# Xneonz0/JPEG-DSP-Studio

Measured on AMD Instinct MI355X. Metric: Mpixels/s forward+inverse pipeline @ Q=50 4:2:0; PSNR vs ref, higher is better.
Workload: dtype f32+f64; 1 GPU; 1920x1080 RGB, Q=50, 4:2:0, prefilter=on, 8x8 blocks (BASELINE configs[1]); global_batch_frames=64, pipeline=serial forward then inverse per step, parallelism=frame-shard x1, world_size=1, quant_table=local (one rank)

## Files before the change

include/jds.h:

```cpp
#ifndef JDS_H
#define JDS_H

#include <stdint.h>

#ifdef __cplusplus
extern "C" {
#endif

#define JDS_ABI_VERSION 3

#define JDS_OK       0
#define JDS_EINVAL  (-1)
#define JDS_ENOTSUP (-2)
#define JDS_EHIP    (-3)
#define JDS_ENOMEM  (-4)

#define JDS_SS_444 0
#define JDS_SS_422 1
#define JDS_SS_420 2
#define JDS_SS_GRAY 3

#define JDS_RUN_SSE 1u
#define JDS_RUN_FWD 2u
#define JDS_RUN_INV 4u
// ... 327 lines not shown
  int64_t rgb_off;
  int64_t H, W;
  int32_t quality;
  int32_t subsampling;
} jds_rgb_item;
int jds_jpeg_quality_info(int32_t quality, int32_t subsampling, int64_t H, int64_t W, jds_jpeg_info* out);
int jds_jpeg_forward_dev(jds_ctx* ctx, const jds_jpeg_info* info, const uint8_t* rgb_dev, int16_t* coeffs_dev,
                         void* stream);
int jds_rgb_to_jpeg(jds_ctx* ctx, const uint8_t* rgb, int32_t rgb_on_device, int64_t H, int64_t W, int32_t quality,
                    int32_t subsampling, int32_t optimize, uint8_t* out, int64_t out_cap, int64_t* out_len);
int jds_rgb_batch_to_jpeg(jds_ctx* ctx, const uint8_t* rgb_base, int32_t rgb_on_device, const jds_rgb_item* items_in,
                          int32_t n, int32_t optimize, uint8_t* out, int64_t out_cap, int32_t out_on_device,
                          jds_jpeg_transcode_item* items_out, int64_t* out_bytes);
int jds_selftest_jpeg_forward(const jds_jpeg_info* info, const uint8_t* rgb, int16_t* coeffs_out);
int jds_selftest_jpeg_fwd_quant(int32_t q, int32_t n, int32_t* out, int32_t* bound);

int jds_selftest_huffdec(const uint8_t* data, int64_t len, int32_t subseq_bits, int16_t* coeffs, int64_t coeffs_cap,
                         int32_t* rounds_out);

int jds_selftest_dct8x8(const double* in, double* out, int64_t n, int32_t inverse);
int jds_selftest_dct16x16(const double* in, double* out, int64_t n, int32_t inverse);

int jds_selftest_fwd32(int32_t subsampling, int32_t prefilter, const double* gauss, const uint8_t* rgb, int64_t H,
                       int64_t W, int32_t plane, int32_t rows_first, float* coeffs, double* bound);
int jds_selftest_fwd16(int32_t subsampling, int32_t prefilter, const double* gauss, const uint8_t* rgb, int64_t H,
                       int64_t W, int32_t plane, int32_t rows_first, float* coeffs, double* bound);

int jds_selftest_inv_fast(int32_t subsampling, const int16_t* coeffs, const double* qtable, int64_t H, int64_t W,
                          int32_t fuse, double* values, uint8_t* bytes);

int jds_selftest_inv_fast16(int32_t subsampling, const int16_t* coeffs, const double* qtable, int64_t H, int64_t W,
                            int32_t fuse, double* values, uint8_t* bytes);

int jds_selftest_inv_rows(int32_t subsampling, int64_t H, int32_t ty, int32_t* out, uint8_t* need);

int jds_selftest_area_tab(int32_t src, int32_t dst, int32_t* n, int32_t* si, double* a);

#ifdef __cplusplus
}
#endif

#endif
```

jpeg-dsp-studio_amd/csrc/jds_abi.hip:

```cpp
#include <algorithm>
#include <mutex>
#include <new>
#include <string>

#include "jds_abi.hpp"
#include "jds_dct16.hpp"
#include "jds_dct8.hpp"

#ifdef JDS_INV6
#define JDS_INV6_LIST 1
#else
#define JDS_INV6_LIST 0
#endif

static const double SSIM_C1 = (0.01 * 255) * (0.01 * 255);
static const double SSIM_C2 = (0.03 * 255) * (0.03 * 255);

thread_local char g_err[512] = "";

constexpr int SSIM_ROWS_MIN = 32;
constexpr size_t SSIM_SCRATCH = (size_t)16 << 30;

static int run_ssim_batch(jds_ctx* c, int items, const uint8_t* const* a, const uint8_t* const* b, int H, int W,
                          double* out, int out_stride, unsigned long long* sse) {
// ... 204 lines not shown

static void fill_geometry(const Geo& G, int mode, jds_geometry* o) {
  o->H = G.H;
  o->W = G.W;
  o->chroma_h = G.hc;
  o->chroma_w = G.wc;
  o->y_blocks_y = G.nby;
  o->y_blocks_x = G.nbx;
  o->c_blocks_y = G.ncy;
  o->c_blocks_x = G.ncx;
  o->coeffs_per_frame = G.cpf;
  o->cb_offset = G.off_cb;
  o->cr_offset = G.off_cr;
  o->tiles = G.tiles_y * G.tiles_x;
  if (G.bs == 16) {
    int my, mx;
    o->threads_fwd = tile_dims16(mode, &my, &mx);
    o->threads_inv = 256;
  } else {
    o->threads_fwd = mode == JDS_SS_420 ? Cfg<M420>::TF : mode == JDS_SS_422 ? Cfg<M422>::TF : Cfg<M444>::TF;
    o->threads_inv = Cfg<M420>::TI;
  }
  o->reserved = 0;
}

static void make_fq(const jds_params* p, FrameQ* q) {
  q->qmax = 0.0;
  q->pad_ = 0.0;
  for (int i = 0; i < 64; ++i) {
    q->q[i] = p->qtable[i];
    q->q16[i] = 16.0 * p->qtable[i];
    q->qmax = q->qmax > p->qtable[i] ? q->qmax : p->qtable[i];
  }
}

static int gen_prepare(const Geo& g, int n_frames, int n, DevBuf& tab, DevBuf& sub, DevBuf& rec, hipStream_t s) {
  const size_t nt = (size_t)g.hc + g.wc;
  AreaTap* h = (AreaTap*)malloc(sizeof(AreaTap) * nt);
  if (!h) return fail(JDS_ENOMEM, "host allocation failed");
  if (area_tab_build(g.H, g.hc, h) < 0 || area_tab_build(g.W, g.wc, h + g.hc) < 0) {
    free(h);
    return fail(JDS_EINVAL, "INTER_AREA table with more than 4 taps per sample (%dx%d)", g.H, g.W);
  }
  hipError_t e = tab.ensure(sizeof(AreaTap) * nt);
  if (e == hipSuccess) e = hipMemcpyAsync(tab.p, h, sizeof(AreaTap) * nt, hipMemcpyHostToDevice, s);
  if (e == hipSuccess) e = hipStreamSynchronize(s);
  free(h);
  HIP_TRY(e);
  HIP_TRY(sub.ensure(sizeof(double) * gen_sub_doubles(g) * (size_t)n_frames));
  HIP_TRY(rec.ensure(sizeof(double) * gen_rec_doubles(g) * (size_t)n));
  return JDS_OK;
}


extern "C" {

int jds_abi_version(void) { return JDS_ABI_VERSION; }

const char* jds_last_error(void) { return g_err; }

int jds_device_count(int* n) {
  if (!n) return fail(JDS_EINVAL, "null argument");
  int c = 0;
  hipError_t e = hipGetDeviceCount(&c);
  if (e != hipSuccess) {
    *n = 0;
// ... 1290 lines not shown
                       int64_t W, int32_t plane, int32_t rows_first, float* coeffs, double* bound) {
  if (!gauss || !rgb || !coeffs || !bound || H < 1 || W < 1 || H > 4096 || W > 4096 || plane < 0 || plane > 2 ||
      subsampling < JDS_SS_444 || subsampling > JDS_SS_420)
    return fail(JDS_EINVAL, "bad argument");
  const bool pf = prefilter != 0 && subsampling != JDS_SS_444;
  double E[512];
  fast_fwd16_bounds(subsampling, pf, gauss, E);
  memcpy(bound, E + (plane ? 256 : 0), 256 * sizeof(double));
  if (fwd16_host_plane(subsampling, pf, gauss, rgb, (int)H, (int)W, plane, rows_first, coeffs))
    return fail(JDS_EINVAL, "plane size must be a multiple of 16");
  return JDS_OK;
}

int jds_selftest_inv_fast(int32_t subsampling, const int16_t* coeffs, const double* qtable, int64_t H, int64_t W,
                          int32_t fuse, double* values, uint8_t* bytes) {
  if (!coeffs || !qtable || !values || !bytes || H < 1 || W < 1 || H > 4096 || W > 4096 ||
      subsampling < JDS_SS_444 || subsampling > JDS_SS_420)
    return fail(JDS_EINVAL, "bad argument");
  if (inv_fast_host(subsampling, coeffs, qtable, (int)H, (int)W, fuse, 8, values, bytes))
    return fail(JDS_EINVAL, "odd chroma geometry: the certified inverse runs even sizes only");
  return JDS_OK;
}

int jds_selftest_inv_fast16(int32_t subsampling, const int16_t* coeffs, const double* qtable, int64_t H, int64_t W,
                            int32_t fuse, double* values, uint8_t* bytes) {
  if (!coeffs || !qtable || !values || !bytes || H < 1 || W < 1 || H > 4096 || W > 4096 ||
      subsampling < JDS_SS_444 || subsampling > JDS_SS_420)
    return fail(JDS_EINVAL, "bad argument");
  if (inv_fast_host(subsampling, coeffs, qtable, (int)H, (int)W, fuse, 16, values, bytes))
    return fail(JDS_EINVAL, "odd chroma geometry: the certified inverse runs even sizes only");
  return JDS_OK;
}

int jds_selftest_area_tab(int32_t src, int32_t dst, int32_t* n, int32_t* si, double* a) {
  if (src < 1 || dst < 1 || dst > src || !n || !si || !a) return fail(JDS_EINVAL, "bad argument");
  AreaTap* t = (AreaTap*)malloc(sizeof(AreaTap) * (size_t)dst);
  if (!t) return fail(JDS_ENOMEM, "host allocation failed");
  if (area_tab_build(src, dst, t) < 0) {
    free(t);
    return fail(JDS_EINVAL, "more than 4 taps per sample");
  }
  for (int d = 0; d < dst; ++d) {
    n[d] = t[d].n;
    for (int k = 0; k < 4; ++k) {
      si[4 * d + k] = k < t[d].n ? t[d].si[k] : -1;
      a[4 * d + k] = k < t[d].n ? t[d].a[k] : 0.0;
    }
  }
  free(t);
  return JDS_OK;
}

int jds_selftest_inv_rows(int32_t subsampling, int64_t H, int32_t ty, int32_t* out, uint8_t* need) {
  if (!out || H < 1 || H > 65536 || ty < 0 || subsampling < JDS_SS_444 || subsampling > JDS_SS_420)
    return fail(JDS_EINVAL, "bad argument");
  int o[8];
  inv_rows(subsampling, (int)H, ty, o);
  for (int i = 0; i < 8; ++i) out[i] = o[i];
  if (need)
    for (int i = 0; i < o[5]; ++i)
      for (int r = 0; r < 8; ++r) need[8 * i + r] = (uint8_t)inv_rows_need(subsampling, (int)H, ty, o[4] + i, r);
  return JDS_OK;
}

int jds_selftest_dct16x16(const double* in, double* out, int64_t n, int32_t inverse) {
  if (!in || !out || n < 0) return fail(JDS_EINVAL, "bad argument");
// ... 18 lines not shown
```

jpeg-dsp-studio_amd/csrc/jds_internal.hpp:

```cpp
#pragma once
#include <hip/hip_runtime.h>
#include <stdint.h>

#include "jds.h"

namespace jds {

enum Mode : int { M444 = JDS_SS_444, M422 = JDS_SS_422, M420 = JDS_SS_420 };

struct Geo {
  int H, W;
  int hc, wc;
  int nby, nbx;
  int ncy, ncx;
  int nmy, nmx;
  int tiles_y, tiles_x, ty_off, tx_off;
  long long cpf;
  long long off_cb, off_cr;
  double up_sy, up_sx;
  int bs;
  int gen;
  int afx, afy;
  int inv_yoff;
};
// ... 16 lines not shown
  int si[4];
  int pad;
  double a[4];
};

struct GenBufs {
  const AreaTap* tabs;
  double* sub;
  double* rec;
};

__host__ __device__ inline int fix_wpi(const Geo& g) { return (int)((g.cpf / 64 + 31) / 32); }

struct Fwd16Fast {
  const void* fq16;
  const float* gk32;
  uint32_t* part;
  uint2* fixlist;
  unsigned* counters;
  int fix_all;
  int parity;
};

struct InvFix {
  unsigned* count;
  unsigned* item;
  int fix_all;
  int parity;
  int rot;
  int probe;
  uint2* list;
};

struct FrameQ {
  double q16[64];
  double q[64];
  double qmax;
  double pad_;
};

template <int MODE>
struct Cfg {
  static constexpr int SY = (MODE == M420) ? 2 : 1;
  static constexpr int SX = (MODE == M444) ? 1 : 2;
  static constexpr int MH = 8 * SY, MW = 8 * SX;
  static constexpr int TH = (MODE == M444) ? 16 : 32;
  static constexpr int TW = 64;
  static constexpr int MY = TH / MH, MX = TW / MW;
  static constexpr int YBR = TH / 8, YBC = TW / 8;
  static constexpr int CBR = TH / MH, CBC = TW / MW;
  static constexpr int NYB = YBR * YBC, NCB = CBR * CBC;
  static constexpr int NB = NYB + 2 * NCB;
  static constexpr int TF = NB * 8;
  static constexpr int RY = (SY == 2) ? 1 : 0, RX = (SX == 2) ? 1 : 0;
  static constexpr int RBR = CBR + 2 * RY, RBC = CBC + 2 * RX;
  static constexpr int NRB = RBR * RBC;
  static constexpr int CWR = 8 * CBR + 2 * RY;
  static constexpr int CWC = 8 * CBC + 2 * RX;
  static constexpr int TI = 384;
};

struct KMarks {
  hipEvent_t* ev = nullptr;
  char (*name)[64] = nullptr;
  int n = 0, cap = 0;
  long long dropped = 0;
};
extern thread_local KMarks* t_kmarks;
void kmark(hipStream_t s, const char* fmt, ...) __attribute__((format(printf, 2, 3)));

__device__ inline void finalize_frame(const Geo& g, jds_frame_stats* s, int zero_bin) {
// ... 34 lines not shown
```

jpeg-dsp-studio_amd/csrc/jds_inv_common.hpp:

```cpp
#pragma once
#include <hip/hip_runtime.h>
#include <stdint.h>

#include "jds_internal.hpp"


namespace jds {

template <int MODE>
struct Inv {
  static constexpr int SY = Cfg<MODE>::SY, SX = Cfg<MODE>::SX;
  static constexpr int TH = (MODE == M420) ? 64 : 32;
  static constexpr int TW = (MODE == M444) ? 64 : 128;
  static constexpr int NT = (MODE == M444) ? 256 : 512;
  static constexpr int RY = (SY == 2) ? 1 : 0, RX = (SX == 2) ? 1 : 0;
  static constexpr int YBC = TW / 8, NYB = (TH / 8) * YBC;
  static constexpr int RB = NT / 8;
  static constexpr int CBR = TH / (8 * SY) + 2 * RY, CBC = TW / (8 * SX) + 2 * RX;
  static constexpr int NCB = CBR * CBC;
  static constexpr int CWR = TH / SY + 2 * RY, CWC = TW / SX + 2 * RX;
  static constexpr int CWS = SX == 2 ? CWC + 4 : CWC;
  static constexpr int NROW = (CBR - 2 * RY) * CBC * 8 + 2 * RY * CBC;
  static constexpr int MB = NCB > RB ? NCB : RB;
  static constexpr int WPE = (MODE == M444) ? 3 : 4;
  static_assert(NCB * 8 <= NT && NROW <= NT && NYB % RB == 0, "one round per chroma plane");
};

template <int MODE>
struct InvRows {
  int y0, cby0, ncbr, cwy0;
  __host__ __device__ __forceinline__ InvRows(int ty, int yoff) {
    using I = Inv<MODE>;
    y0 = ty * I::TH - yoff;
    cby0 = ty * (I::TH / (8 * I::SY)) - I::RY;
    ncbr = I::CBR - (yoff ? 1 : 0);
    cwy0 = y0 / I::SY - I::RY;
  }
  __host__ __device__ __forceinline__ bool need(int by, int r) const {
    return !Inv<MODE>::RY || (unsigned)(by * 8 + r - cwy0) < (unsigned)Inv<MODE>::CWR;
  }
};

constexpr int MS = 72;

__device__ __forceinline__ int tslot(int r, int c) { return r * 8 + ((((c >> 1) ^ (r & 3)) << 1) | (c & 1)); }

struct Col16 {
  int16_t q[8];
};
__device__ __forceinline__ Col16 load_col(const int16_t* __restrict__ plane, long long boff, int v, bool ok) {
  const int16_t* blk = plane + (ok ? boff : 0ll);
  Col16 c;
#pragma unroll
  for (int r = 0; r < 8; ++r) c.q[r] = blk[r * 8 + v];
  return c;
}

#ifdef JDS_INV6
typedef short jds_short2 __attribute__((ext_vector_type(2)));
struct Col16p {
  jds_short2 w[4];
  __device__ __forceinline__ int q(int r) const { return (int)((r & 1) ? w[r >> 1].y : w[r >> 1].x); }
};
__device__ __forceinline__ Col16p load_colp(const int16_t* __restrict__ plane, long long boff, int v, bool ok) {
  const int16_t* blk = plane + (ok ? boff : 0ll);
  Col16p c;
#pragma unroll
  for (int i = 0; i < 4; ++i) {
    c.w[i].x = blk[(2 * i) * 8 + v];
    c.w[i].y = blk[(2 * i + 1) * 8 + v];
  }
  return c;
}

__device__ __forceinline__ uint4 load_rowq(const int16_t* __restrict__ plane, long long boff, int k, bool ok) {
  return *reinterpret_cast<const uint4*>(plane + (ok ? boff : 0ll) + 8 * k);
}
__device__ __forceinline__ uint4 load_rowq_b(__amdgpu_buffer_rsrc_t r, long long boff, int k, bool ok) {
  typedef unsigned u4 __attribute__((ext_vector_type(4)));
  const u4 v = __builtin_amdgcn_raw_buffer_load_b128(r, (int)(((ok ? boff : 0ll) + 8 * k) * 2), 0, 0);
  return make_uint4(v.x, v.y, v.z, v.w);
}
__device__ __forceinline__ Col16p xpose_q16(uint4 v) {
  uint32_t w[4] = {v.x, v.y, v.z, v.w};
#pragma unroll
  for (int i = 0; i < 2; ++i) {
    const auto a = __builtin_amdgcn_permlane32_swap(w[i], w[i + 2], false, false);
// ... 68 lines not shown
```

jpeg-dsp-studio_amd/csrc/jds_inv_fast.hip:

```cpp
#include <hip/hip_runtime.h>
#include <stdint.h>
#include <string.h>

#include <algorithm>
#include <cmath>
#include <vector>

#include "jds_device.hpp"
#include "jds_internal.hpp"
#include "jds_inv_common.hpp"
#include "jds_inv_exact.hpp"
#include "jds_inv16_exact.hpp"

#pragma clang fp contract(fast)

namespace jds {

constexpr double K_LIN = 8.762155e-13 * 1.01;
constexpr double K_CONST = 1.024801e-12 * 1.01;
constexpr double K_LIN16 = 3.345910e-12 * 1.01;
constexpr double K_CONST16 = 1.024801e-12 * 1.01;

#define JDS_AAN_LIST                                                                                 \
  1.0, 0x1.63150b15e8536p+0, 0x1.4e7ae9144f0fcp+0, 0x1.2d062ef88e319p+0, 1.0, 0x1.92469c0dcf32dp-1, \
// ... 32 lines not shown
  const double o11 = (z11 - z13) * F_SQ2;
  const double z5 = (z10 + z12) * F_A2C2;
  const double o10 = M::mad(-z12, F_K10, z5);
  const double o12 = M::mad(-z10, F_K12, z5);
  const double o6 = o12 - o7, o5 = o11 - o6, o4 = o10 - o5;
  v[0] = e0 + o7;
  v[7] = e0 - o7;
  v[1] = e1 + o6;
  v[6] = e1 - o6;
  v[2] = e2 + o5;
  v[5] = e2 - o5;
  v[3] = e3 + o4;
  v[4] = e3 - o4;
}

template <class M = MadDev>
__host__ __device__ __forceinline__ double fvsum(double a, double b) { return M::mad(b, 3.0, a); }
template <class M = MadDev>
__host__ __device__ __forceinline__ double fhsum(double far, double near) { return M::mad(near, 3.0, far); }
template <int SH>
constexpr double USC = SH == 0 ? 1.0 : (SH == 2 ? 0.25 : 0.0625);
template <int SY, int SX>
constexpr int USH = (SY == 2 ? 2 : 0) + (SX == 2 ? 2 : 0);

template <class M = MadDev, int SH = 0>
__host__ __device__ __forceinline__ double col_b(double yv, double cb) { return M::mad(cb, 1.772 * USC<SH>, yv); }
template <class M = MadDev, int SH = 0>
__host__ __device__ __forceinline__ double col_gt(double yv, double cb) { return M::mad(cb, -0.344136 * USC<SH>, yv); }
template <class M = MadDev, int SH = 0>
__host__ __device__ __forceinline__ double col_r(double yv, double cr) { return M::mad(cr, 1.402 * USC<SH>, yv); }
template <class M = MadDev, int SH = 0>
__host__ __device__ __forceinline__ double col_g(double gt, double cr) { return M::mad(cr, -0.714136 * USC<SH>, gt); }

constexpr int QS_STRIDE = 10;
constexpr int QS_WORDS = 1 ? 8 * QS_STRIDE : 64;
__device__ __forceinline__ int qs_index(int r, int v) { return 1 ? v * QS_STRIDE + r : r * 8 + v; }
__device__ __forceinline__ void fast_col(const Col16& in, const double* __restrict__ qs, int v,
                                         double* __restrict__ dst, int& qhi, int& qlo) {
  double c[8];
  double t[8];
#pragma unroll
  for (int p = 0; p < 4; ++p) {
    const double2 d = *reinterpret_cast<const double2*>(qs + v * QS_STRIDE + 2 * p);
    t[2 * p] = d.x;
    t[2 * p + 1] = d.y;
  }
#pragma unroll
  for (int r = 0; r < 8; ++r) {
    const double qd = (double)in.q[r];
    qhi = max(qhi, (int)in.q[r]);
    qlo = min(qlo, (int)in.q[r]);
    c[r] = qd * t[r];
  }
  aan8(c);
#pragma unroll
  for (int r = 0; r < 8; ++r) dst[tslot(r, v)] = c[r];
}

template <int LO = 0, bool CLIP = true>
__device__ __forceinline__ void fast_row(const double* __restrict__ src, int u, double (&c)[8]) {
  const int sw = u & 3;
#pragma unroll
  for (int p = 0; p < 4; ++p) {
    const double2 d = *reinterpret_cast<const double2*>(src + u * 8 + 2 * (p ^ sw));
    c[2 * p] = d.x;
    c[2 * p + 1] = d.y;
  }
  aan8(c);
  if constexpr (CLIP) {
#pragma unroll
    for (int k = 0; k < 8; ++k) c[k] = fmin(fmax(c[k], (double)LO), (double)(LO + 255));
  }
}

template <int MODE>
__device__ __forceinline__ void chroma8_fast(const double* __restrict__ cw, int x0, int cwx0, int wq, int wt,
                                             double (&C)[8]) {
  using I = Inv<MODE>;
  if constexpr (I::SX == 1) {
#pragma unroll
    for (int k = 0; k < 8; ++k) C[k] = cw[wq * I::CWS + x0 + k - cwx0];
  } else {
    const int c0 = x0 / 2 - 1 - cwx0;
    double vb[6];
#pragma unroll
    for (int j = 0; j < 6; ++j) {
      if constexpr (I::SY == 2)
        vb[j] = fvsum(cw[wq * I::CWS + c0 + j], cw[wt * I::CWS + c0 + j]);
      else
        vb[j] = cw[wq * I::CWS + c0 + j];
    }
#pragma unroll
    for (int i = 0; i < 4; ++i) {
      C[2 * i] = fhsum(vb[i], vb[i + 1]);
      C[2 * i + 1] = fhsum(vb[i + 2], vb[i + 1]);
    }
  }
}

constexpr double MAGIC = 0x1.8p+20;
constexpr uint32_t MAGIC_HI = 0x41380000u;

__device__ __forceinline__ uint32_t byte_cert_y(double y, uint32_t& lo_min, uint32_t& lo_max) {
  const uint32_t lo = (uint32_t)__double2loint(y), hi = (uint32_t)__double2hiint(y);
  lo_min = lo_min < lo ? lo_min : lo;
  lo_max = lo_max > lo ? lo_max : lo;
  const uint32_t c = hi < MAGIC_HI ? MAGIC_HI : hi;
  return c > MAGIC_HI + 255u ? MAGIC_HI + 255u : c;
}

__device__ __forceinline__ uint32_t cert_hi(double y, uint32_t& lo_min, uint32_t& lo_max) {
  const uint32_t lo = (uint32_t)__double2loint(y), hi = (uint32_t)__double2hiint(y);
  lo_min = lo_min < lo ? lo_min : lo;
  lo_max = lo_max > lo ? lo_max : lo;
  return hi;
}
// ... 2 lines not shown
  asm("v_sat_pk_u8_i16 %0, %1" : "=v"(r) : "v"(x));
  return r;
}
__device__ __forceinline__ uint32_t pack4s(uint32_t a, uint32_t b, uint32_t c, uint32_t d) {
  const uint32_t ab = sat_pk_u8_i16(__builtin_amdgcn_perm(b, a, 0x05040100u));
  const uint32_t cd = sat_pk_u8_i16(__builtin_amdgcn_perm(d, c, 0x05040100u));
  return ab | (cd << 16);
}

__device__ __forceinline__ uint32_t pack4(uint32_t a, uint32_t b, uint32_t c, uint32_t d) {
  const uint32_t ab = __builtin_amdgcn_perm(b, a, 0x0c0c0400u);
  const uint32_t cd = __builtin_amdgcn_perm(d, c, 0x04000c0cu);
  return ab | cd;
}

template <int SH>
__device__ __forceinline__ void cert_row_step(uint32_t& mn, uint32_t& mx, uint32_t& qm) {
  const uint32_t a = (uint32_t)__builtin_amdgcn_update_dpp((int)0xffffffff, (int)mn, 0x110 + SH, 0xf, 0xf, false);
  const uint32_t b = (uint32_t)__builtin_amdgcn_update_dpp(0, (int)mx, 0x110 + SH, 0xf, 0xf, false);
  const uint32_t c = (uint32_t)__builtin_amdgcn_update_dpp(0, (int)qm, 0x110 + SH, 0xf, 0xf, false);
  mn = mn < a ? mn : a;
  mx = mx > b ? mx : b;
  qm = qm > c ? qm : c;
}
__device__ __forceinline__ void cert_to_lds(uint32_t mn, uint32_t mx, uint32_t qm, uint32_t* s_cert) {
  cert_row_step<1>(mn, mx, qm);
  cert_row_step<2>(mn, mx, qm);
  cert_row_step<4>(mn, mx, qm);
  cert_row_step<8>(mn, mx, qm);
  if ((threadIdx.x & 15) == 15) {
    atomicMin(&s_cert[0], mn);
    atomicMax(&s_cert[1], mx);
    atomicMax(&s_cert[2], qm);
  }
}

template <int MODE, int XTRA>
__device__ __forceinline__ bool inv_fast_tile(InvShared<MODE, XTRA>& sh, const Geo& g, const int tiles_x,
                                              const int frame, const int tile, const int16_t* __restrict__ coeffs,
                                              const FrameQ* __restrict__ fq, const uint8_t* __restrict__ rgb_in,
                                              uint8_t* __restrict__ rgb_out, jds_frame_stats* __restrict__ st,
                                              double* __restrict__ sse_y_part, unsigned* __restrict__ fixcount,
                                              unsigned* __restrict__ next_count, unsigned* __restrict__ cnt_now,
                                              const int in_div, const int fix_all) {
  using I = Inv<MODE>;
  constexpr int USH_ = USH<I::SY, I::SX>;
  double* s_mid = sh.mid;
  double (*s_cw)[I::CWR * I::CWS] = sh.cw;
  __shared__ __attribute__((aligned(16))) double s_qs[QS_WORDS];
  __shared__ double s_qmax;
  __shared__ double s_red[I::NT / 64], s_dq[I::NT / 64];
  __shared__ uint32_t s_lmin[I::NT / 64], s_lmax[I::NT / 64];
  __shared__ uint32_t s_cert[3];
  __shared__ double s_dummy[64];
  __shared__ unsigned long long s_sse;
  const int tid = threadIdx.x, lv = tid & 7, lb = tid >> 3;
  const int ty = tile / tiles_x, tx = tile - ty * tiles_x;
  const InvRows<MODE> rows(ty, g.inv_yoff);
  const int Y0 = rows.y0, X0 = tx * I::TW;
  const int16_t* cf = coeffs + (size_t)frame * g.cpf;
  int qhi = 0, qlo = 0;

  const int cby0 = rows.cby0, cbx0 = X0 / (8 * I::SX) - I::RX;
  const int cwy0 = rows.cwy0, cwx0 = X0 / I::SX - I::RX;
  auto luma_blk = [&](int r, int& by, int& bx) {
    const int blk = r * I::RB + lb;
    const int bi = blk / I::YBC, bj = blk - bi * I::YBC;
    by = Y0 / 8 + bi;
    bx = X0 / 8 + bj;
    return by >= 0 && by < g.nby && bx < g.nbx;
  };
  auto table_setup = [&]() {
    if (tid < 64) {
      const double q = fq[frame].q[tid];
      s_qs[qs_index(tid >> 3, tid & 7)] = q * c_aan[tid >> 3] * c_aan[tid & 7] * 0.125;
      if (tid == 0) {
        s_cert[0] = 0xffffffffu;
        s_cert[1] = 0u;
        s_cert[2] = 0u;
      }
    }
    if (XTRA && tid == 0) s_sse = 0ull;
    __syncthreads();
  };
  Col16 lq;
  {
    int by, bx;
    const bool ok = luma_blk(0, by, bx);
    lq = load_col(cf, ((long long)by * g.nbx + bx) * 64, lv, ok);
  }
  auto chroma_task = [&](const int p, const int by, const int bx, const Col16& cur) {
    const bool need = rows.need(by, lv);
    fast_col(cur, s_qs, lv, s_mid + lb * MS, qhi, qlo);
    if (need) {
      double c[8];
      fast_row<-128>(s_mid + lb * MS, lv, c);
      double* w = &s_cw[p][(by * 8 + lv - cwy0) * I::CWS];
      const int wc0 = bx * 8 - cwx0;
#pragma unroll
      for (int k = 0; k < 8; ++k)
        *((unsigned)(wc0 + k) < (unsigned)I::CWC ? w + wc0 + k : s_dummy + (tid & 63)) = c[k];
      if constexpr (I::SX == 2) {
        if (bx == 0 && wc0 >= 1) w[wc0 - 1] = c[0];
        const int ke = g.wc - 1 - bx * 8;
        if ((unsigned)ke < 8u) {
          const double e = (ke == 0 ? c[0] : ke == 1 ? c[1] : ke == 2 ? c[2] : ke == 3 ? c[3]
                            : ke == 4 ? c[4] : ke == 5 ? c[5] : ke == 6 ? c[6] : c[7]);
          for (int col = wc0 + ke + 1; col < I::CWC; ++col) w[col] = e;
        }
      }
    }
  };
  constexpr bool MIXP = 1 && MODE == M422 && 2 * I::NCB > I::RB && 2 * I::NCB <= 2 * I::RB;
  if constexpr (MIXP) {
    constexpr int NTASK = 2 * I::NCB;
    auto tinfo = [&](int tt, int& pp, int& ii, int& by, int& bx, bool& ok) -> long long {
      pp = tt >= I::NCB ? 1 : 0;
      const int b = tt - pp * I::NCB;
      ii = b / I::CBC;
      const int jj = b - ii * I::CBC;
      by = cby0 + ii;
      bx = cbx0 + jj;
      ok = tt < NTASK && by >= 0 && bx >= 0 && by < g.ncy && bx < g.ncx;
      return ((long long)by * g.ncx + bx) * 64;
    };
    int pp, ii, by, bx;
    bool ok;
    long long off = tinfo(lb, pp, ii, by, bx, ok);
    Col16 cq = load_col(cf + (pp ? g.off_cr : g.off_cb), off, lv, ok);
    table_setup();
    if (tid == 0) s_qmax = fq[frame].qmax;
#pragma unroll 1
    for (int tt = lb; tt < NTASK; tt += I::RB) {
      const Col16 cur = cq;
      const int pc = pp, byc = by, bxc = bx;
      const bool okc = ok;
      if (tt + I::RB < NTASK) {
        off = tinfo(tt + I::RB, pp, ii, by, bx, ok);
        cq = load_col(cf + (pp ? g.off_cr : g.off_cb), off, lv, ok);
      }
      if (okc) chroma_task(pc, byc, bxc, cur);
    }
  } else {
    const bool ctask = lb < rows.ncbr * I::CBC;
    const int ci = lb / I::CBC, cj = lb - ci * I::CBC;
    const int cby = cby0 + ci, cbx = cbx0 + cj;
    const bool cvalid = ctask && cby >= 0 && cbx >= 0 && cby < g.ncy && cbx < g.ncx;
    const long long cboff = ((long long)cby * g.ncx + cbx) * 64;
    Col16 cq = load_col(cf + g.off_cb, cboff, lv, cvalid);
    table_setup();
    if (tid == 0) s_qmax = fq[frame].qmax;
    if (ctask) {
#pragma unroll 1
      for (int p = 0; p < 2; ++p) {
        const Col16 cur = cq;
        if (p == 0) cq = load_col(cf + g.off_cr, cboff, lv, cvalid);
        if (cvalid) chroma_task(p, cby, cbx, cur);
      }
    }
  }
  __syncthreads();

  uint32_t lo_min = 0xffffffffu, lo_max = 0u;
  unsigned long long sse = 0ull;
  double ssy = 0.0;
  const uint8_t* in_f = XTRA ? rgb_in + (size_t)(frame / in_div) * g.H * g.W * 3 : nullptr;
  uint8_t* out_f = rgb_out + (size_t)frame * g.H * g.W * 3;
#pragma unroll 1
  for (int r = 0; r < I::NYB / I::RB; ++r) {
    int by, bx;
    const bool bvalid = luma_blk(r, by, bx);
    unsigned long long r_sse = 0ull;
    double r_ssy = 0.0;
    const Col16 cur = lq;
    if (r + 1 < I::NYB / I::RB) {
      int by1, bx1;
      const bool ok1 = luma_blk(r + 1, by1, bx1);
      lq = load_col(cf, ((long long)by1 * g.nbx + bx1) * 64, lv, ok1);
    }
    if (bvalid) fast_col(cur, s_qs, lv, s_mid + lb * MS, qhi, qlo);
    const int y = by * 8 + lv, x0 = bx * 8;
    if (bvalid && y < g.H && x0 < g.W) {
      double Yv[8];
      fast_row<-128>(s_mid + lb * MS, lv, Yv);
      int wq, wt = 0;
      if constexpr (I::SY == 2) {
        const int m = y >> 1;
        const int rq = (y & 1) ? m + 1 : m - 1;
        wq = clampi(clampi(rq, 0, g.hc - 1) - cwy0, 0, I::CWR - 1);
        wt = clampi(clampi(m, 0, g.hc - 1) - cwy0, 0, I::CWR - 1);
      } else {
        wq = y - cwy0;
      }
      const int nx = g.W - x0 < 8 ? g.W - x0 : 8;
      uint8_t* o = out_f + ((size_t)y * g.W + x0) * 3;
      const bool wide = nx == 8 && ((((uintptr_t)o) & 7u) == 0);
      uint32_t in[6] = {0u, 0u, 0u, 0u, 0u, 0u};
      if constexpr (XTRA > 0) {
        const uint8_t* src = in_f + ((size_t)y * g.W + x0) * 3;
        if (wide) {
          const uint2* s2 = reinterpret_cast<const uint2*>(src);
          const uint2 a = s2[0], b2 = s2[1], c = s2[2];
          in[0] = a.x; in[1] = a.y; in[2] = b2.x; in[3] = b2.y; in[4] = c.x; in[5] = c.y;
        } else {
#pragma unroll
          for (int k = 0; k < 24; ++k)
            if (k < 3 * nx) in[k >> 2] |= (uint32_t)src[k] << (8 * (k & 3));
        }
      }
      uint32_t pk[6];
      uint32_t r_min = 0xffffffffu, r_max = 0u;
      {
        uint32_t cb[24];
        double C[8], Gt[8];
        chroma8_fast<MODE>(s_cw[0], x0, cwx0, wq, wt, C);
#pragma unroll
        for (int k = 0; k < 8; ++k) {
          Yv[k] = Yv[k] + (MAGIC + 128.0);
          const double B = col_b<MadDev, USH_>(Yv[k], C[k]);
          Gt[k] = col_gt<MadDev, USH_>(Yv[k], C[k]);
          cb[3 * k + 2] = cert_hi(B, r_min, r_max);
        }
        chroma8_fast<MODE>(s_cw[1], x0, cwx0, wq, wt, C);
#pragma unroll
        for (int k = 0; k < 8; ++k) {
          const double R = col_r<MadDev, USH_>(Yv[k], C[k]);
          const double G = col_g<MadDev, USH_>(Gt[k], C[k]);
          cb[3 * k] = cert_hi(R, r_min, r_max);
          cb[3 * k + 1] = cert_hi(G, r_min, r_max);
        }
#pragma unroll
        for (int w = 0; w < 6; ++w) pk[w] = pack4s(cb[4 * w], cb[4 * w + 1], cb[4 * w + 2], cb[4 * w + 3]);
      }
      lo_min = lo_min < r_min ? lo_min : r_min;
      lo_max = lo_max > r_max ? lo_max : r_max;
      if (wide) {
        uint2* o2 = reinterpret_cast<uint2*>(o);
        o2[0] = make_uint2(pk[0], pk[1]);
        o2[1] = make_uint2(pk[2], pk[3]);
        o2[2] = make_uint2(pk[4], pk[5]);
      } else {
#pragma unroll
        for (int b = 0; b < 24; ++b)
          if (b < 3 * nx) o[b] = (uint8_t)(pk[b >> 2] >> (8 * (b & 3)));
      }
      if constexpr (XTRA > 0) {
        auto byte_of = [](const uint32_t (&w)[6], int b) { return (int)((w[b >> 2] >> (8 * (b & 3))) & 255u); };
#pragma unroll
        for (int k = 0; k < 8; ++k) {
          if (k < nx) {
            const int b = 3 * k;
            const int o0 = byte_of(in, b), o1 = byte_of(in, b + 1), o2 = byte_of(in, b + 2);
            const int ur = byte_of(pk, b), ug = byte_of(pk, b + 1), ub = byte_of(pk, b + 2);
            const int d0 = o0 - ur, d1 = o1 - ug, d2 = o2 - ub;
            r_sse += (unsigned long long)(d0 * d0 + d1 * d1 + d2 * d2);
            r_ssy = r_ssy + luma_sse_e6(d0, d1, d2);
          }
        }
      }
    }
    if constexpr (XTRA > 0) {
      sse += r_sse;
      ssy = ssy + r_ssy;
    }
  }

  int qm = max(qhi, -qlo);
  cert_to_lds(lo_min, lo_max, (uint32_t)qm, s_cert);
  if constexpr (XTRA > 0) {
    unsigned long long s = sse;
#pragma unroll
    for (int o = 32; o > 0; o >>= 1) s += __shfl_xor(s, o, 64);
    if ((tid & 63) == 0) atomicAdd(&s_sse, s);
    double d = ssy;
#pragma unroll
    for (int o = 32; o > 0; o >>= 1) d = d + __shfl_xor(d, o, 64);
    if ((tid & 63) == 0) s_red[tid >> 6] = d;
  }
  __syncthreads();
  if (tid == 0) {
    const uint32_t mn = s_cert[0], mx = s_cert[1];
    const double q = (double)s_cert[2];
    const double E = K_LIN * (q * s_qmax) + K_CONST + 0x1p-31;
    const double T = ceil(E * 0x1p+32) + 1.0;
    const bool uncertain = (double)mn <= T || (double)mx >= 0x1p+32 - 1.0 - T;
    sh.redo = uncertain || fix_all;
    if (sh.redo) {
      atomicAdd(fixcount, 1u);
      atomicAdd(cnt_now + frame, 1u);
    } else if constexpr (XTRA > 0) {
      double a = 0.0;
      for (int i = 0; i < I::NT / 64; ++i) a = a + s_red[i];
      sse_y_part[(size_t)frame * gridDim.x + tile] = a;
      atomicAdd((unsigned long long*)&st[frame].sse_rgb, s_sse);
    }
    if (frame == 0 && tile == 0) *next_count = 0u;
  }
  __syncthreads();
  return sh.redo != 0;
}

template <int MODE, int XTRA>
__global__ void __launch_bounds__(Inv<MODE>::NT) __attribute__((amdgpu_waves_per_eu(Inv<MODE>::WPE)))
k_inv_fast(const Geo g, const int tiles_x, const int16_t* __restrict__ coeffs, const FrameQ* __restrict__ fq,
           const uint8_t* __restrict__ rgb_in, uint8_t* __restrict__ rgb_out, jds_frame_stats* __restrict__ st,
           double* __restrict__ sse_y_part, unsigned* __restrict__ fixcount, unsigned* __restrict__ next_count,
           unsigned* __restrict__ item_cnt, const int rot, const int probe, const int in_div, const int fix_all,
           const int fin) {
  __shared__ __attribute__((aligned(16))) InvShared<MODE, XTRA> sh;
#ifdef JDS_PROBE_LDS_PAD
  __shared__ unsigned s_pad[JDS_PROBE_LDS_PAD];
  if (threadIdx.x == 0) s_pad[blockIdx.x % JDS_PROBE_LDS_PAD] = 0u;
#endif
  const int tid = threadIdx.x;
  const int frame = blockIdx.y, tile = blockIdx.x;
  if (fin >= 0 && tile == 0 && tid == 0) finalize_frame(g, st + frame, fin);
  const unsigned n_items = gridDim.y, ntile = gridDim.x;
  unsigned* cnt_prev = item_cnt + ((rot + 2) % 3) * n_items;
// ... 748 lines not shown
    kmark(s, "k_inv_fast<%d,1>", MODE);
    return hipGetLastError();
  }
  hipLaunchKernelGGL((k_inv_fast<MODE, 0>), grid, blk, 0, s, g, tx, coeffs, fq, nullptr, rgb_out, st, part, cnt, nxt,
                     fx.item, fx.rot, fx.probe, in_div, fx.fix_all, fin);
  kmark(s, "k_inv_fast<%d,0>", MODE);
  return hipGetLastError();
}

hipError_t launch_inv_fast(int mode, const Geo& g, int n, const int16_t* coeffs, const FrameQ* fq,
                           const uint8_t* rgb_in, uint8_t* rgb_out, jds_frame_stats* st, double* part,
                           const InvFix& fx, hipStream_t s, int in_div, int fin) {
  switch (mode) {
    case M420: return inv_fast_t<M420>(g, n, coeffs, fq, rgb_in, rgb_out, st, part, fx, s, in_div, fin);
    case M422: return inv_fast_t<M422>(g, n, coeffs, fq, rgb_in, rgb_out, st, part, fx, s, in_div, fin);
    default: {
      (void)rgb_in;
      (void)part;
      (void)in_div;
      const long long nblk = (long long)g.nby * g.nbx;
      const dim3 grid((unsigned)((nblk + 8 * I444_WAVES - 1) / (8 * I444_WAVES)), n), blk(64 * I444_WAVES);
      hipLaunchKernelGGL(k_inv_fast444, grid, blk, 0, s, g, coeffs, fq, rgb_out, st, fx.count + fx.parity,
                         fx.count + (fx.parity ^ 1), fx.item, fx.rot, fx.fix_all, fin);
      kmark(s, "k_inv_fast444");
      return hipGetLastError();
    }
  }
}

template <class M, int BS>
static void inv_fast_host_t(int mode, const int16_t* cf, const double* Q, int H, int W, double* vout,
                            uint8_t* bout) {
  const int sy = mode == M420 ? 2 : 1, sx = mode == M444 ? 1 : 2;
  double qs[64];
  for (int i = 0; i < 64; ++i) qs[i] = Q[i] * h_aan[i >> 3] * h_aan[i & 7] * 0.125;
  auto deq = [&](int q, int u, int v) {
    if constexpr (BS == 8) return (double)q * qs[u * 8 + v];
    return ((double)(q * (int)Q[(u >> 1) * 8 + (v >> 1)]) * s16_of(h_aan, u)) * s16_of(h_aan, v);
  };
  auto line = [](double(&c)[BS]) {
    if constexpr (BS == 8)
      aan8<M>(c);
    else
      fidct16<M>(c);
  };
  std::vector<double> pl[3];
  int ph[3], pw[3], st[3];
  size_t off = 0;
  for (int p = 0; p < 3; ++p) {
    ph[p] = p ? H / sy : H;
    pw[p] = p ? W / sx : W;
    const int nby = (ph[p] + BS - 1) / BS, nbx = (pw[p] + BS - 1) / BS;
    st[p] = nbx * BS;
    pl[p].assign((size_t)nby * BS * st[p], 0.0);
    for (int by = 0; by < nby; ++by)
      for (int bx = 0; bx < nbx; ++bx) {
        const int16_t* b = cf + off + ((size_t)by * nbx + bx) * BS * BS;
        double mid[BS][BS];
        for (int v = 0; v < BS; ++v) {
          double c[BS];
          for (int r = 0; r < BS; ++r) c[r] = deq(b[r * BS + v], r, v);
          line(c);
          for (int r = 0; r < BS; ++r) mid[r][v] = c[r];
        }
        for (int u = 0; u < BS; ++u) {
          double c[BS];
          for (int k = 0; k < BS; ++k) c[k] = mid[u][k];
          line(c);
          for (int k = 0; k < BS; ++k)
            pl[p][(size_t)(by * BS + u) * st[p] + bx * BS + k] = fmin(fmax(c[k], -128.0), 127.0);
// ... 71 lines not shown
```

jpeg-dsp-studio_amd/jds/_abi.py:

```python
from __future__ import annotations

import ctypes as C
import importlib.util
import os
import threading

import numpy as np

_HERE = os.path.dirname(os.path.abspath(__file__))
LIB_PATH = os.environ.get('JDS_LIB_PATH') or os.path.join(_HERE, 'libjds.so')

JDS_OK, JDS_EINVAL, JDS_ENOTSUP, JDS_EHIP, JDS_ENOMEM = 0, -1, -2, -3, -4
SS_444, SS_422, SS_420 = 0, 1, 2
MODE_CODES = {'4:4:4': SS_444, '4:2:2': SS_422, '4:2:0': SS_420}
SS_GRAY = 3
JPEG_MODE_CODES = dict(MODE_CODES, gray=SS_GRAY)
RENDER_CODES = {'reference': 0, 'libjpeg': 1}
RUN_SSE, RUN_FWD, RUN_INV, RUN_EXACT, RUN_EXACT_INV, RUN_INV_FIXALL, RUN_FWD_FIXALL, RUN_INV_FAST = 1, 2, 4, 8, 16, 32, 64, 128


SCALE_DENOMS = (1, 2, 4, 8)


def scale_denom_arg(scale_denom, render=None) -> int:
# ... 223 lines not shown
                                  C.POINTER(C.c_int64)]),
    'jds_jpeg_transcode': (C.c_int, [_P, _P, C.c_int64, C.c_int32, _P, C.c_int64, C.POINTER(C.c_int64),
                                     C.POINTER(JpegInfo)]),
    'jds_jpeg_batch_transcode': (C.c_int, [_P, _P, _P, C.c_int32, C.c_int32, _P, C.c_int64, C.c_int32,
                                           C.POINTER(JpegTranscodeItem), C.POINTER(C.c_int64)]),
    'jds_selftest_jpeg_transcode': (C.c_int, [_P, C.c_int64, C.c_int32, _P, C.c_int64, C.POINTER(C.c_int64)]),
    'jds_selftest_jpeg_encode': (C.c_int, [C.POINTER(JpegInfo), _P, C.c_int32, _P, C.c_int64, _P, C.c_int64,
                                           C.POINTER(C.c_int64)]),
    'jds_selftest_jpeg_hist_dev': (C.c_int, [_P, C.POINTER(JpegInfo), _P, _P]),
    'jds_jpeg_transform_info': (C.c_int, [_P, C.c_int64, C.c_int32, C.POINTER(C.c_int32), C.POINTER(C.c_int64),
                                          C.POINTER(C.c_int64)]),
    'jds_jpeg_transform': (C.c_int, [_P, _P, C.c_int64, C.c_int32, C.c_int32, _P, C.c_int64, C.POINTER(C.c_int64),
                                     C.POINTER(JpegInfo)]),
    'jds_jpeg_batch_transform': (C.c_int, [_P, _P, _P, C.c_int32, _P, C.c_int32, _P, C.c_int64, C.c_int32,
                                           C.POINTER(JpegTranscodeItem), C.POINTER(C.c_int64)]),
    'jds_selftest_jpeg_transform': (C.c_int, [_P, C.c_int64, C.c_int32, C.c_int32, _P, C.c_int64,
                                              C.POINTER(C.c_int64)]),
    'jds_selftest_coef_transform_dev': (C.c_int, [_P, C.POINTER(JpegInfo), C.c_int32, _P, _P]),
    'jds_jpeg_quality_info': (C.c_int, [C.c_int32, C.c_int32, C.c_int64, C.c_int64, C.POINTER(JpegInfo)]),
    'jds_jpeg_forward_dev': (C.c_int, [_P, C.POINTER(JpegInfo), _P, _P, _P]),
    'jds_rgb_to_jpeg': (C.c_int, [_P, _P, C.c_int32, C.c_int64, C.c_int64, C.c_int32, C.c_int32, C.c_int32, _P,
                                  C.c_int64, C.POINTER(C.c_int64)]),
    'jds_rgb_batch_to_jpeg': (C.c_int, [_P, _P, C.c_int32, C.POINTER(RgbItem), C.c_int32, C.c_int32, _P, C.c_int64,
                                        C.c_int32, C.POINTER(JpegTranscodeItem), C.POINTER(C.c_int64)]),
    'jds_selftest_jpeg_forward': (C.c_int, [C.POINTER(JpegInfo), _P, _P]),
    'jds_selftest_jpeg_fwd_quant': (C.c_int, [C.c_int32, C.c_int32, _P, C.POINTER(C.c_int32)]),
    'jds_selftest_jpeg_window': (C.c_int, [C.c_int32, C.c_int32, C.c_int32, C.c_int32, C.c_int32, _P]),
    'jds_selftest_dct8x8': (C.c_int, [_P, _P, C.c_int64, C.c_int32]),
    'jds_selftest_dct16x16': (C.c_int, [_P, _P, C.c_int64, C.c_int32]),
    'jds_selftest_area_tab': (C.c_int, [C.c_int32, C.c_int32, _P, _P, _P]),
    'jds_selftest_inv_rows': (C.c_int, [C.c_int32, C.c_int64, C.c_int32, _P, _P]),
    'jds_selftest_inv_fast': (C.c_int, [C.c_int32, _P, _P, C.c_int64, C.c_int64, C.c_int32, _P, _P]),
    'jds_selftest_inv_fast16': (C.c_int, [C.c_int32, _P, _P, C.c_int64, C.c_int64, C.c_int32, _P, _P]),
    'jds_selftest_fwd32': (C.c_int, [C.c_int32, C.c_int32, _P, _P, C.c_int64, C.c_int64, C.c_int32, C.c_int32, _P,
                                     _P]),
    'jds_selftest_fwd16': (C.c_int, [C.c_int32, C.c_int32, _P, _P, C.c_int64, C.c_int64, C.c_int32, C.c_int32, _P,
                                     _P]),
}
_OPTIONAL_SIGS: dict = {}

_lib = None
_lock = threading.Lock()


def _preload_torch_hip():
    spec = importlib.util.find_spec('torch')
    if spec is None or not spec.submodule_search_locations:
        return None
    cand = os.path.join(list(spec.submodule_search_locations)[0], 'lib', 'libamdhip64.so')
    if os.path.exists(cand):
        return C.CDLL(cand, mode=C.RTLD_GLOBAL)
    return None


def lib():
    global _lib
    if _lib is not None:
        return _lib
    with _lock:
        if _lib is not None:
            return _lib
        if not os.path.exists(LIB_PATH):
            raise ImportError(f'{LIB_PATH} is missing: build it with `python -c "import __graft_entry__ as g; '
                              f'g.build()"` (hipcc --offload-arch=gfx950)')
        _preload_torch_hip()
        h = C.CDLL(LIB_PATH, mode=C.RTLD_GLOBAL)
# ... 180 lines not shown
```

Baseline: 229,200 Mpixels/s.

## Prefold dequant table on host, per-wave LDS copies, 32-bit indexing, DPP cert reduce

The AAN-scaled dequant table is now folded once on the host into FrameQ, and each wavefront copies it into its own LDS slice. This replaces the per-block recompute and uses a wave barrier instead of a block-wide __syncthreads. Coefficient loads and output addressing switch to 32-bit offsets. Chroma window addressing is simplified by precomputing row and column bases, with one block column kept fixed per lane. The certificate min/max reduction is merged into one value reduced with DPP row shuffles before the LDS atomics. In exchange the code uses more LDS, assumes offsets fit in 32 bits, and removes a block barrier between table setup and use, which relies on later syncs for s_cert init ordering.

```diff
diff --git a/include/jds.h b/include/jds.h
--- a/include/jds.h
+++ b/include/jds.h
@@ -383,6 +383,8 @@
 int jds_selftest_inv_fast16(int32_t subsampling, const int16_t* coeffs, const double* qtable, int64_t H, int64_t W,
                             int32_t fuse, double* values, uint8_t* bytes);
 
+int jds_selftest_inv_fold(const double* qtable, double* folded);
+
 int jds_selftest_inv_rows(int32_t subsampling, int64_t H, int32_t ty, int32_t* out, uint8_t* need);
 
 int jds_selftest_area_tab(int32_t src, int32_t dst, int32_t* n, int32_t* si, double* a);
diff --git a/jpeg-dsp-studio_amd/csrc/jds_abi.hip b/jpeg-dsp-studio_amd/csrc/jds_abi.hip
--- a/jpeg-dsp-studio_amd/csrc/jds_abi.hip
+++ b/jpeg-dsp-studio_amd/csrc/jds_abi.hip
@@ -260,6 +260,7 @@
     q->q16[i] = 16.0 * p->qtable[i];
     q->qmax = q->qmax > p->qtable[i] ? q->qmax : p->qtable[i];
   }
+  inv_fold_table(q->q, q->qs);
 }
 
 static int gen_prepare(const Geo& g, int n_frames, int n, DevBuf& tab, DevBuf& sub, DevBuf& rec, hipStream_t s) {
@@ -1616,6 +1617,16 @@
   return JDS_OK;
 }
 
+int jds_selftest_inv_fold(const double* qtable, double* folded) {
+  if (!qtable || !folded) return fail(JDS_EINVAL, "bad argument");
+  jds_params p{};
+  memcpy(p.qtable, qtable, sizeof(p.qtable));
+  FrameQ fq;
+  make_fq(&p, &fq);
+  for (int i = 0; i < 64; ++i) folded[i] = fq.qs[qs_index(i >> 3, i & 7)];
+  return JDS_OK;
+}
+
 int jds_selftest_area_tab(int32_t src, int32_t dst, int32_t* n, int32_t* si, double* a) {
   if (src < 1 || dst < 1 || dst > src || !n || !si || !a) return fail(JDS_EINVAL, "bad argument");
   AreaTap* t = (AreaTap*)malloc(sizeof(AreaTap) * (size_t)dst);
diff --git a/jpeg-dsp-studio_amd/csrc/jds_internal.hpp b/jpeg-dsp-studio_amd/csrc/jds_internal.hpp
--- a/jpeg-dsp-studio_amd/csrc/jds_internal.hpp
+++ b/jpeg-dsp-studio_amd/csrc/jds_internal.hpp
@@ -72,11 +72,17 @@
   uint2* list;
 };
 
+constexpr int QS_STRIDE = 10;
+constexpr int QS_WORDS = 8 * QS_STRIDE;
+__host__ __device__ inline int qs_index(int r, int v) { return v * QS_STRIDE + r; }
+void inv_fold_table(const double* Q, double* qs);
+
 struct FrameQ {
   double q16[64];
   double q[64];
   double qmax;
   double pad_;
+  double qs[QS_WORDS];
 };
 
 template <int MODE>
diff --git a/jpeg-dsp-studio_amd/csrc/jds_inv_common.hpp b/jpeg-dsp-studio_amd/csrc/jds_inv_common.hpp
--- a/jpeg-dsp-studio_amd/csrc/jds_inv_common.hpp
+++ b/jpeg-dsp-studio_amd/csrc/jds_inv_common.hpp
@@ -53,6 +53,16 @@
   Col16 c;
 #pragma unroll
   for (int r = 0; r < 8; ++r) c.q[r] = blk[r * 8 + v];
+  return c;
+}
+
+__device__ __forceinline__ Col16 load_col32(const int16_t* __restrict__ frame, unsigned plane, unsigned boff, int v,
+                                            bool ok) {
+  const unsigned o = (plane + (ok ? boff : 0u) + (unsigned)v) * 2u;
+  const char* b = reinterpret_cast<const char*>(frame);
+  Col16 c;
+#pragma unroll
+  for (int r = 0; r < 8; ++r) c.q[r] = *reinterpret_cast<const int16_t*>(b + (size_t)o + r * 16);
   return c;
 }
 
diff --git a/jpeg-dsp-studio_amd/csrc/jds_inv_fast.hip b/jpeg-dsp-studio_amd/csrc/jds_inv_fast.hip
--- a/jpeg-dsp-studio_amd/csrc/jds_inv_fast.hip
+++ b/jpeg-dsp-studio_amd/csrc/jds_inv_fast.hip
@@ -88,9 +88,6 @@
 template <class M = MadDev, int SH = 0>
 __host__ __device__ __forceinline__ double col_g(double gt, double cr) { return M::mad(cr, -0.714136 * USC<SH>, gt); }
 
-constexpr int QS_STRIDE = 10;
-constexpr int QS_WORDS = 1 ? 8 * QS_STRIDE : 64;
-__device__ __forceinline__ int qs_index(int r, int v) { return 1 ? v * QS_STRIDE + r : r * 8 + v; }
 __device__ __forceinline__ void fast_col(const Col16& in, const double* __restrict__ qs, int v,
                                          double* __restrict__ dst, int& qhi, int& qlo) {
   double c[8];
@@ -113,6 +110,11 @@
   for (int r = 0; r < 8; ++r) dst[tslot(r, v)] = c[r];
 }
 
+void inv_fold_table(const double* Q, double* qs) {
+  for (int i = 0; i < QS_WORDS; ++i) qs[i] = 0.0;
+  for (int i = 0; i < 64; ++i) qs[qs_index(i >> 3, i & 7)] = Q[i] * h_aan[i >> 3] * h_aan[i & 7] * 0.125;
+}
+
 template <int LO = 0, bool CLIP = true>
 __device__ __forceinline__ void fast_row(const double* __restrict__ src, int u, double (&c)[8]) {
   const int sw = u & 3;
@@ -130,14 +132,12 @@
 }
 
 template <int MODE>
-__device__ __forceinline__ void chroma8_fast(const double* __restrict__ cw, int x0, int cwx0, int wq, int wt,
-                                             double (&C)[8]) {
+__device__ __forceinline__ void chroma8_fast(const double* __restrict__ cw, int c0, int wq, int wt, double (&C)[8]) {
   using I = Inv<MODE>;
   if constexpr (I::SX == 1) {
 #pragma unroll
-    for (int k = 0; k < 8; ++k) C[k] = cw[wq * I::CWS + x0 + k - cwx0];
+    for (int k = 0; k < 8; ++k) C[k] = cw[wq * I::CWS + c0 + k];
   } else {
-    const int c0 = x0 / 2 - 1 - cwx0;
     double vb[6];
 #pragma unroll
     for (int j = 0; j < 6; ++j) {
@@ -206,6 +206,25 @@
     atomicMin(&s_cert[0], mn);
     atomicMax(&s_cert[1], mx);
     atomicMax(&s_cert[2], qm);
+  }
+}
+
+template <int SH>
+__device__ __forceinline__ void cert2_row_step(uint32_t& d, uint32_t& qm) {
+  const uint32_t a = (uint32_t)__builtin_amdgcn_update_dpp((int)0xffffffff, (int)d, 0x110 + SH, 0xf, 0xf, false);
+  const uint32_t c = (uint32_t)__builtin_amdgcn_update_dpp(0, (int)qm, 0x110 + SH, 0xf, 0xf, false);
+  d = d < a ? d : a;
+  qm = qm > c ? qm : c;
+}
+__device__ __forceinline__ void cert2_to_lds(uint32_t mn, uint32_t mx, uint32_t qm, uint32_t* s_cert) {
+  uint32_t d = mn < ~mx ? mn : ~mx;
+  cert2_row_step<1>(d, qm);
+  cert2_row_step<2>(d, qm);
+  cert2_row_step<4>(d, qm);
+  cert2_row_step<8>(d, qm);
+  if ((threadIdx.x & 15) == 15) {
+    atomicMin(&s_cert[0], d);
+    atomicMax(&s_cert[1], qm);
   }
 }
 
@@ -221,11 +240,10 @@
   constexpr int USH_ = USH<I::SY, I::SX>;
   double* s_mid = sh.mid;
   double (*s_cw)[I::CWR * I::CWS] = sh.cw;
-  __shared__ __attribute__((aligned(16))) double s_qs[QS_WORDS];
+  __shared__ __attribute__((aligned(16))) double s_qs_all[I::NT / 64][QS_WORDS];
   __shared__ double s_qmax;
-  __shared__ double s_red[I::NT / 64], s_dq[I::NT / 64];
-  __shared__ uint32_t s_lmin[I::NT / 64], s_lmax[I::NT / 64];
-  __shared__ uint32_t s_cert[3];
+  __shared__ double s_red[I::NT / 64];
+  __shared__ uint32_t s_cert[2];
   __shared__ double s_dummy[64];
   __shared__ unsigned long long s_sse;
   const int tid = threadIdx.x, lv = tid & 7, lb = tid >> 3;
@@ -236,44 +254,53 @@
   int qhi = 0, qlo = 0;
 
   const int cby0 = rows.cby0, cbx0 = X0 / (8 * I::SX) - I::RX;
-  const int cwy0 = rows.cwy0, cwx0 = X0 / I::SX - I::RX;
+  const int cwy0 = rows.cwy0;
+  const int lbj = lb % I::YBC;
+  static_assert(I::RB % I::YBC == 0, "a lane keeps its block column over the rounds");
   auto luma_blk = [&](int r, int& by, int& bx) {
     const int blk = r * I::RB + lb;
-    const int bi = blk / I::YBC, bj = blk - bi * I::YBC;
+    const int bi = blk / I::YBC, bj = lbj;
     by = Y0 / 8 + bi;
     bx = X0 / 8 + bj;
     return by >= 0 && by < g.nby && bx < g.nbx;
   };
+  double* const s_qs = s_qs_all[tid >> 6];
   auto table_setup = [&]() {
-    if (tid < 64) {
-      const double q = fq[frame].q[tid];
-      s_qs[qs_index(tid >> 3, tid & 7)] = q * c_aan[tid >> 3] * c_aan[tid & 7] * 0.125;
-      if (tid == 0) {
-        s_cert[0] = 0xffffffffu;
-        s_cert[1] = 0u;
-        s_cert[2] = 0u;
-      }
-    }
-    if (XTRA && tid == 0) s_sse = 0ull;
-    __syncthreads();
+    const int l = tid & 63;
+    if (l < QS_WORDS / 2)
+      reinterpret_cast<double2*>(s_qs)[l] = reinterpret_cast<const double2*>(fq[frame].qs)[l];
+    __builtin_amdgcn_fence(__ATOMIC_RELEASE, "wavefront");
+    __builtin_amdgcn_wave_barrier();
+    __builtin_amdgcn_fence(__ATOMIC_ACQUIRE, "wavefront");
+    if (tid == 0) {
+      s_cert[0] = 0xffffffffu;
+      s_cert[1] = 0u;
+      s_qmax = fq[frame].qmax;
+      if (XTRA) s_sse = 0ull;
+    }
   };
   Col16 lq;
   {
     int by, bx;
     const bool ok = luma_blk(0, by, bx);
-    lq = load_col(cf, ((long long)by * g.nbx + bx) * 64, lv, ok);
-  }
-  auto chroma_task = [&](const int p, const int by, const int bx, const Col16& cur) {
-    const bool need = rows.need(by, lv);
+    lq = load_col32(cf, 0u, (unsigned)(by * g.nbx + bx) * 64u, lv, ok);
+  }
+  const int wr_off = g.inv_yoff / I::SY - 7 * I::RY;
+  auto chroma_task = [&](const int p, const int wr0, const int wc0, const int bx, const Col16& cur) {
+    const int wr = wr0 + lv;
+    const bool need = !I::RY || (unsigned)wr < (unsigned)I::CWR;
     fast_col(cur, s_qs, lv, s_mid + lb * MS, qhi, qlo);
     if (need) {
       double c[8];
       fast_row<-128>(s_mid + lb * MS, lv, c);
-      double* w = &s_cw[p][(by * 8 + lv - cwy0) * I::CWS];
-      const int wc0 = bx * 8 - cwx0;
-#pragma unroll
-      for (int k = 0; k < 8; ++k)
-        *((unsigned)(wc0 + k) < (unsigned)I::CWC ? w + wc0 + k : s_dummy + (tid & 63)) = c[k];
+      double* w = &s_cw[p][wr * I::CWS];
+      const bool in_lo = !I::RX || wc0 >= 0, in_hi = !I::RX || wc0 + 7 < I::CWC;
+      static_assert(!I::RX || (I::CWC - 2) % 8 == 0, "the window: whole blocks and one ring column each side");
+#pragma unroll
+      for (int k = 0; k < 8; ++k) {
+        const bool in = k == 0 ? in_lo : k == 7 ? in_hi : (in_lo && in_hi);
+        *(in ? w + wc0 + k : s_dummy + (tid & 63)) = c[k];
+      }
       if constexpr (I::SX == 2) {
         if (bx == 0 && wc0 >= 1) w[wc0 - 1] = c[0];
         const int ke = g.wc - 1 - bx * 8;
@@ -288,7 +315,7 @@
   constexpr bool MIXP = 1 && MODE == M422 && 2 * I::NCB > I::RB && 2 * I::NCB <= 2 * I::RB;
   if constexpr (MIXP) {
     constexpr int NTASK = 2 * I::NCB;
-    auto tinfo = [&](int tt, int& pp, int& ii, int& by, int& bx, bool& ok) -> long long {
+    auto tinfo = [&](int tt, int& pp, int& ii, int& by, int& bx, bool& ok) -> unsigned {
       pp = tt >= I::NCB ? 1 : 0;
       const int b = tt - pp * I::NCB;
       ii = b / I::CBC;
@@ -296,14 +323,15 @@
       by = cby0 + ii;
       bx = cbx0 + jj;
       ok = tt < NTASK && by >= 0 && bx >= 0 && by < g.ncy && bx < g.ncx;
-      return ((long long)by * g.ncx + bx) * 64;
+      return (unsigned)(by * g.ncx + bx) * 64u;
     };
+    const unsigned pcb = (unsigned)g.off_cb, pcr = (unsigned)g.off_cr;
+    const int cwx0 = X0 / I::SX - I::RX;
     int pp, ii, by, bx;
     bool ok;
-    long long off = tinfo(lb, pp, ii, by, bx, ok);
-    Col16 cq = load_col(cf + (pp ? g.off_cr : g.off_cb), off, lv, ok);
+    unsigned off = tinfo(lb, pp, ii, by, bx, ok);
+    Col16 cq = load_col32(cf, pp ? pcr : pcb, off, lv, ok);
     table_setup();
-    if (tid == 0) s_qmax = fq[frame].qmax;
 #pragma unroll 1
     for (int tt = lb; tt < NTASK; tt += I::RB) {
       const Col16 cur = cq;
@@ -311,25 +339,24 @@
       const bool okc = ok;
       if (tt + I::RB < NTASK) {
         off = tinfo(tt + I::RB, pp, ii, by, bx, ok);
-        cq = load_col(cf + (pp ? g.off_cr : g.off_cb), off, lv, ok);
-      }
-      if (okc) chroma_task(pc, byc, bxc, cur);
+        cq = load_col32(cf, pp ? pcr : pcb, off, lv, ok);
+      }
+      if (okc) chroma_task(pc, byc * 8 - cwy0, bxc * 8 - cwx0, bxc, cur);
     }
   } else {
     const bool ctask = lb < rows.ncbr * I::CBC;
     const int ci = lb / I::CBC, cj = lb - ci * I::CBC;
     const int cby = cby0 + ci, cbx = cbx0 + cj;
     const bool cvalid = ctask && cby >= 0 && cbx >= 0 && cby < g.ncy && cbx < g.ncx;
-    const long long cboff = ((long long)cby * g.ncx + cbx) * 64;
-    Col16 cq = load_col(cf + g.off_cb, cboff, lv, cvalid);
+    const unsigned cboff = (unsigned)(cby * g.ncx + cbx) * 64u;
+    Col16 cq = load_col32(cf, (unsigned)g.off_cb, cboff, lv, cvalid);
     table_setup();
-    if (tid == 0) s_qmax = fq[frame].qmax;
     if (ctask) {
 #pragma unroll 1
       for (int p = 0; p < 2; ++p) {
         const Col16 cur = cq;
-        if (p == 0) cq = load_col(cf + g.off_cr, cboff, lv, cvalid);
-        if (cvalid) chroma_task(p, cby, cbx, cur);
+        if (p == 0) cq = load_col32(cf, (unsigned)g.off_cr, cboff, lv, cvalid);
+        if (cvalid) chroma_task(p, ci * 8 + wr_off, cj * 8 - 7 * I::RX, cbx, cur);
       }
     }
   }
@@ -350,7 +377,7 @@
     if (r + 1 < I::NYB / I::RB) {
       int by1, bx1;
       const bool ok1 = luma_blk(r + 1, by1, bx1);
-      lq = load_col(cf, ((long long)by1 * g.nbx + bx1) * 64, lv, ok1);
+      lq = load_col32(cf, 0u, (unsigned)(by1 * g.nbx + bx1) * 64u, lv, ok1);
     }
     if (bvalid) fast_col(cur, s_qs, lv, s_mid + lb * MS, qhi, qlo);
     const int y = by * 8 + lv, x0 = bx * 8;
@@ -367,11 +394,12 @@
         wq = y - cwy0;
       }
       const int nx = g.W - x0 < 8 ? g.W - x0 : 8;
-      uint8_t* o = out_f + ((size_t)y * g.W + x0) * 3;
-      const bool wide = nx == 8 && ((((uintptr_t)o) & 7u) == 0);
+      const unsigned po = (unsigned)(y * g.W + x0) * 3u;
+      uint8_t* o = out_f + po;
+      const bool wide = nx == 8 && (((unsigned)(uintptr_t)out_f + po) & 7u) == 0;
       uint32_t in[6] = {0u, 0u, 0u, 0u, 0u, 0u};
       if constexpr (XTRA > 0) {
-        const uint8_t* src = in_f + ((size_t)y * g.W + x0) * 3;
+        const uint8_t* src = in_f + po;
         if (wide) {
           const uint2* s2 = reinterpret_cast<const uint2*>(src);
           const uint2 a = s2[0], b2 = s2[1], c = s2[2];
@@ -387,7 +415,7 @@
       {
         uint32_t cb[24];
         double C[8], Gt[8];
-        chroma8_fast<MODE>(s_cw[0], x0, cwx0, wq, wt, C);
+        chroma8_fast<MODE>(s_cw[0], lbj * (8 / I::SX), wq, wt, C);
 #pragma unroll
         for (int k = 0; k < 8; ++k) {
           Yv[k] = Yv[k] + (MAGIC + 128.0);
@@ -395,7 +423,7 @@
           Gt[k] = col_gt<MadDev, USH_>(Yv[k], C[k]);
           cb[3 * k + 2] = cert_hi(B, r_min, r_max);
         }
-        chroma8_fast<MODE>(s_cw[1], x0, cwx0, wq, wt, C);
+        chroma8_fast<MODE>(s_cw[1], lbj * (8 / I::SX), wq, wt, C);
 #pragma unroll
         for (int k = 0; k < 8; ++k) {
           const double R = col_r<MadDev, USH_>(Yv[k], C[k]);
@@ -440,7 +468,7 @@
   }
 
   int qm = max(qhi, -qlo);
-  cert_to_lds(lo_min, lo_max, (uint32_t)qm, s_cert);
+  cert2_to_lds(lo_min, lo_max, (uint32_t)qm, s_cert);
   if constexpr (XTRA > 0) {
     unsigned long long s = sse;
 #pragma unroll
@@ -453,11 +481,11 @@
   }
   __syncthreads();
   if (tid == 0) {
-    const uint32_t mn = s_cert[0], mx = s_cert[1];
-    const double q = (double)s_cert[2];
+    const uint32_t d = s_cert[0];
+    const double q = (double)s_cert[1];
     const double E = K_LIN * (q * s_qmax) + K_CONST + 0x1p-31;
     const double T = ceil(E * 0x1p+32) + 1.0;
-    const bool uncertain = (double)mn <= T || (double)mx >= 0x1p+32 - 1.0 - T;
+    const bool uncertain = (double)d <= T;
     sh.redo = uncertain || fix_all;
     if (sh.redo) {
       atomicAdd(fixcount, 1u);
@@ -1272,10 +1300,10 @@
 static void inv_fast_host_t(int mode, const int16_t* cf, const double* Q, int H, int W, double* vout,
                             uint8_t* bout) {
   const int sy = mode == M420 ? 2 : 1, sx = mode == M444 ? 1 : 2;
-  double qs[64];
-  for (int i = 0; i < 64; ++i) qs[i] = Q[i] * h_aan[i >> 3] * h_aan[i & 7] * 0.125;
+  double qs[QS_WORDS];
+  inv_fold_table(Q, qs);
   auto deq = [&](int q, int u, int v) {
-    if constexpr (BS == 8) return (double)q * qs[u * 8 + v];
+    if constexpr (BS == 8) return (double)q * qs[qs_index(u, v)];
     return ((double)(q * (int)Q[(u >> 1) * 8 + (v >> 1)]) * s16_of(h_aan, u)) * s16_of(h_aan, v);
   };
   auto line = [](double(&c)[BS]) {
diff --git a/jpeg-dsp-studio_amd/jds/_abi.py b/jpeg-dsp-studio_amd/jds/_abi.py
--- a/jpeg-dsp-studio_amd/jds/_abi.py
+++ b/jpeg-dsp-studio_amd/jds/_abi.py
@@ -279,6 +279,7 @@
     'jds_selftest_inv_rows': (C.c_int, [C.c_int32, C.c_int64, C.c_int32, _P, _P]),
     'jds_selftest_inv_fast': (C.c_int, [C.c_int32, _P, _P, C.c_int64, C.c_int64, C.c_int32, _P, _P]),
     'jds_selftest_inv_fast16': (C.c_int, [C.c_int32, _P, _P, C.c_int64, C.c_int64, C.c_int32, _P, _P]),
+    'jds_selftest_inv_fold': (C.c_int, [_P, _P]),
     'jds_selftest_fwd32': (C.c_int, [C.c_int32, C.c_int32, _P, _P, C.c_int64, C.c_int64, C.c_int32, C.c_int32, _P,
                                      _P]),
     'jds_selftest_fwd16': (C.c_int, [C.c_int32, C.c_int32, _P, _P, C.c_int64, C.c_int64, C.c_int32, C.c_int32, _P,
```

New measurement: 230,700 Mpixels/s, median of 6. About the same (+0.7%).
